# datastryio/weaviate

Measured on AMD Instinct MI355X. Metric: batched 10-NN QPS at recall@10≥0.95, 1M×128-d L2, on 1/2/4/8 MI355X, higher is better.
Workload: dtype f32 (f16 MFMA keys certified by an error bound, f32 reference-order re-rank)

## Files before the change

weaviate_amd/csrc/wv_api.hip:

```cpp
#include <hip/hip_runtime.h>
#include <hipcub/hipcub.hpp>

#include <algorithm>
#include <array>
#include <atomic>
#include <chrono>
#include <cmath>
#include <cstdio>
#include <cstdlib>
#include <condition_variable>
#include <cstring>
#include <mutex>
#include <string>
#include <vector>

#include "../../include/wvgpu.h"
#include "wv_device.h"

#include "wv_params.h"

extern "C" {
hipError_t wv_launch_bf_mfma(const wv::BfParams* p, hipStream_t s);
hipError_t wv_launch_bf_finalize(const wv::BfFinParams* p, hipStream_t s);
hipError_t wv_launch_bf_finalize_wide(const wv::BfFinParams* p, hipStream_t s);
// ... 567 lines not shown
        excl = ix->cexcl.as<uint64_t>();
        allow = nullptr;
    }
    if (ix->metric == WV_L2_SQUARED)
        HIP_TRY(wv_launch_h16_xns(xnorm, ntl * tile_rows, ix->h16_sx, ix->qscale.as<float>(), ix->xns.as<float>(), s));
    wv::H16Params hp{};
    hp.X = ximg;
    hp.rowidx = wd ? rowidx : nullptr;
    hp.Q = ix->qimg16.p;
    hp.xns = ix->xns.as<float>();
    hp.excl = excl;
    hp.allow = allow;
    hp.qscale = ix->qscale.as<float>();
    hp.sx = ix->h16_sx;
    hp.N = N;
    hp.nq = nq;
    hp.metric = ix->metric;
    hp.n_qblocks = nqb;
    hp.wide_rows = 128;
    hp.clean_tiles = wd ? 0 : rowidx ? N / wv::H_BN : allow ? 0 : std::min<uint64_t>(ix->clean_words, N / wv::H_BN);
    hp.locality = 1;
    wv::BfFinParams fp{};
    fp.X = ix->vecs.as<float>();
    fp.Q = d_q;
    fp.qnorm = ix->q_nrm2.as<float>();
    fp.xnorm_max = ix->maxnorm_host;
    fp.nq = nq;
    fp.D = ix->dim;
    fp.ldx = ix->ldx;
    fp.ldq = ix->dpad;
    fp.metric = ix->metric;
    fp.k = k;
    fp.id_base = ix->cfg.id_base;
    fp.out_ids = d_out_ids;
    fp.out_d = d_out_d;
    fp.out_n = d_out_n;
    fp.fail = ix->fail.as<int32_t>();
    fp.fail_thr = ix->fail_thr.as<float>();
    fp.bq = bq;
    fp.prod = prod;
    fp.kp = kp;
    fp.h16 = 1;
    hp.ns = ns;
    fp.qscale = ix->qscale.as<float>();
    fp.sx = ix->h16_sx;
    fp.ex_max = ix->h16_ex;
    fp.qres = ix->qres.as<float>();
    const bool wide = k > wv::FIN_KF;
    auto target = [&](uint64_t tiles) {
        uint64_t t = (uint64_t)ix->n_cus * wg_per_cu;
        if (wide) t = std::max<uint64_t>(t, (uint64_t)nqb * std::min<uint64_t>(tiles, (uint64_t)k + 2));
        return (int)std::min<uint64_t>(t, 1u << 30);
    };
    int sample = wv::H_SAMPLE;
    if (const char* e = std::getenv("WV_H16_SAMPLE")) sample = std::max(1, std::atoi(e));
    const bool seed = !wd && ntl >= 64 * (uint64_t)sample && !std::getenv("WV_H16_NO_SEED");
    const uint64_t nts = seed ? (ntl + sample - 1) / sample : 0;
    wv::BfSchedule ss{};
    if (seed) ss = wv::bf_schedule(nq, nts * wv::H_BN, target(nts), bq, wv::H_BN);
    const bool seed_lists = seed && !wide && !n_dev && k <= 64 &&
                            (uint64_t)ss.n_slots * wv::H_PROD * wv::BF_KP <= 256 && std::getenv("WV_H16_SEED_LISTS");
    const uint64_t ntl_main = seed_lists ? ntl - nts : ntl;
    wv::BfSchedule sch{};
    if (n_dev) {
        if (!wd || wide) return fail(WV_ESTATE, "run_h16: device-counted rows need the wide-D pass");
        const int S = std::max(1, target(ntl) / nqb);
        sch.bq = bq;
        sch.ntiles = (uint64_t)S;
        sch.units_per_block = 1;
        sch.n_blocks = nqb * S;
        sch.n_slots = S + 1;
    }
    if (wd && !wide && sch.n_blocks == 0) sch = wv::bf_schedule_aligned(nq, N, target(ntl), bq, tile_rows, false);
    if (sch.n_blocks == 0)
        sch = wv::bf_schedule(nq, seed_lists ? ntl_main * tile_rows : N, target(ntl_main), bq, tile_rows);
    if (wide && (uint64_t)sch.n_slots * prod * kp > (uint64_t)wv::FINW_NE)
        return fail(WV_ESTATE, "run_h16: too many lists for the wide finalize");
    const int out_slots = sch.n_slots + (seed_lists ? 1 : 0);
    HIP_TRY(ix->cand_d.ensure((size_t)nq * out_slots * prod * kp * 4));
    HIP_TRY(ix->cand_id.ensure((size_t)nq * out_slots * prod * kp * 4));
    auto seed_minima = [&](int stride) -> int {
        const uint64_t nt = (ntl + stride - 1) / stride;
        const wv::BfSchedule ms = wv::bf_schedule(nq, nt * wv::H_BN, target(nt), bq, wv::H_BN);
        HIP_TRY(ix->cand_d.ensure((size_t)nq * std::max(ms.n_slots * seed_prod, out_slots * prod * kp) * 4));
        hp.ntiles = ms.ntiles;
        hp.ntiles_real = ms.ntiles;
        hp.units_per_block = ms.units_per_block;
        hp.n_slots = ms.n_slots;
        hp.tile_stride = stride;
        hp.tile_base = 0;
        hp.tau = nullptr;
        hp.out_d = ix->cand_d.as<float>();
        hp.out_id = nullptr;
        HIP_TRY(wv_launch_bf_h16(&hp, ns, 1, s));
        wv::H16SeedParams sp{};
        sp.minima = ix->cand_d.as<float>();
        sp.n_slots = ms.n_slots;
        sp.ntiles = ms.ntiles;
        sp.units_per_block = ms.units_per_block;
        sp.nq = nq;
        sp.k = k;
        sp.metric = ix->metric;
        sp.D = ix->dim;
        sp.qscale = ix->qscale.as<float>();
        sp.sx = ix->h16_sx;
        sp.qnorm = ix->q_nrm2.as<float>();
        sp.xnorm_max = ix->maxnorm_host;
        sp.ex_max = ix->h16_ex;
        sp.qres = ix->qres.as<float>();
// ... 2 lines not shown
        sp.bq = bq;
        sp.prod = seed_prod;
        if (seed_lists) {
            HIP_TRY(wv_launch_h16_seed(&sp, s));
            HIP_TRY(ix->seed_d.ensure((size_t)nq * ss.n_slots * prod * kp * 4));
            HIP_TRY(ix->seed_id.ensure((size_t)nq * ss.n_slots * prod * kp * 4));
            hp.ntiles = ss.ntiles;
            hp.ntiles_real = ss.ntiles;
            hp.units_per_block = ss.units_per_block;
            hp.n_slots = ss.n_slots;
            hp.tile_stride = 1;
            hp.tile_base = ntl_main;
            hp.tau = ix->tau.as<float>();
            hp.out_d = ix->seed_d.as<float>();
            hp.out_id = ix->seed_id.as<uint32_t>();
            HIP_TRY(wv_launch_bf_h16(&hp, ns, 0, s));
            hp.tile_base = 0;
            hp.tau = nullptr;
            sp.minima = ix->seed_d.as<float>();
            sp.ids = ix->seed_id.as<uint32_t>();
            sp.n_slots = ss.n_slots;
            sp.ntiles = ss.ntiles;
            sp.units_per_block = ss.units_per_block;
            sp.prod = prod * kp;
            sp.out_d = ix->cand_d.as<float>();
            sp.out_id = ix->cand_id.as<uint32_t>();
            sp.out_slots = out_slots;
            sp.out_ntiles = sch.ntiles;
            sp.out_upb = sch.units_per_block;
        }
        HIP_TRY(wv_launch_h16_seed(&sp, s));
        return WV_OK;
    };
    if (seed) {
        TREC(6);
        int mult = 4;
        if (const char* e = std::getenv("WV_H16_LIST_MULT")) mult = std::max(1, std::atoi(e));
        if (int rc = seed_minima(seed_lists ? mult * sample : sample)) return rc;
        TREC(7);
    }
    hp.ntiles = sch.ntiles;
    hp.ntiles_real = ntl_main;
    hp.out_slots = seed_lists ? out_slots : 0;
    hp.units_per_block = sch.units_per_block;
    hp.n_slots = sch.n_slots;
    hp.n_dev = n_dev;
    hp.tile_stride = 1;
    hp.tau = nullptr;
    if (!seed) HIP_TRY(hipMemsetAsync(ix->gtau.p, 0xFF, (size_t)nq * 4, s));
    hp.gtau = ix->gtau.as<unsigned int>();
    hp.kth = k <= (wd ? 2 * kp : prod * kp) && !seed && !std::getenv("WV_H16_NO_RUNNING")
                 ? k
                 : 0;
    const char* xe = std::getenv("WV_H16_XSLOT");
    const bool xs_on = !xe || std::atoi(xe) != 0;
    if (xs_on && !wd && 2 * sch.n_slots <= 32 && k <= 2 * sch.n_slots) {
        const size_t gb = (size_t)nq * 2 * sch.n_slots * 4;
        HIP_TRY(ix->gslot.ensure(gb));
        HIP_TRY(hipMemsetAsync(ix->gslot.p, 0x7F, gb, s));
        hp.gslot = ix->gslot.as<float>();
        hp.xslot = 1;
        hp.kth = k;
    }
    if (hp.kth) {
        HIP_TRY(ix->marg.ensure((size_t)nq * 4));
        HIP_TRY(wv_launch_h16_margin(ix->metric, ix->dim, ix->q_nrm2.as<float>(), ix->qres.as<float>(),
                                     ix->maxnorm_host, ix->h16_ex, ix->h16_sx, ix->qscale.as<float>(), nq,
                                     ix->marg.as<float>(), s));
        hp.marg = ix->marg.as<float>();
    }
    hp.out_d = ix->cand_d.as<float>();
    hp.out_id = ix->cand_id.as<uint32_t>();
    const bool rotate = !wd && nqb >= 2 && sch.ntiles == ntl_main;
    if (rotate) hp.locality |= 2;
    if (int rc = block_order(ix, (uint64_t)nqb, sch, s, &hp.block_order, rotate)) return rc;
    TREC(0);
    HIP_TRY(wd ? wv_launch_bf_h16w(&hp, s) : wv_launch_bf_h16(&hp, ns, 0, s));
    TREC(1);
    if (rowidx && wide)
        HIP_TRY(wv_launch_remap_ids(ix->cand_id.as<uint32_t>(), nq, sch.n_slots, prod * kp, bq, sch.ntiles,
                                    sch.units_per_block, rowidx, N, n_dev, s));
    if (rowidx && !wide) {
        fp.rowidx = rowidx;
        fp.rowidx_n = N;
        fp.rowidx_ndev = n_dev;
    }
    fp.cand_d = ix->cand_d.as<float>();
    fp.cand_id = ix->cand_id.as<uint32_t>();
    fp.n_slots = out_slots;
    fp.extra_slot = seed_lists ? 1 : 0;
    fp.ntiles = sch.ntiles;
    fp.units_per_block = sch.units_per_block;
    HIP_TRY(wv_launch_h16_gtau(ix->gtau.as<unsigned int>(), nq, ix->h16_sx, ix->qscale.as<float>(), ix->tau.as<float>(),
                               s));
    fp.tau_in = ix->tau.as<float>();
    TREC(2);
    HIP_TRY(wide ? wv_launch_bf_finalize_wide(&fp, s) : wv_launch_bf_finalize(&fp, s));
    TREC(3);
    (void)fails;
    return WV_OK;
}

int queue_fbd(wv_index* ix, const float* d_q, int nq, int k, const uint64_t* d_allow, uint64_t allow_nbits,
              uint64_t allow_stride, uint64_t* d_out_ids, float* d_out_d, int32_t* d_out_n, hipStream_t s) {
    const uint64_t N = ix->n_rows;
    HIP_TRY(ix->fbd_list.ensure((size_t)nq * 4));
    HIP_TRY(ix->fbd_nf.ensure(16));
    HIP_TRY(ix->fbd_over.ensure((size_t)nq * 4));
    HIP_TRY(ix->fbd_cd.ensure((size_t)nq * wv::FB_CAP * 4));
// ... 2013 lines not shown
```

weaviate_amd/csrc/wv_h16.hip:

```cpp
#include "wv_device.h"
#include "wv_params.h"
#include "wv_topk.h"

#include <float.h>

#include "wv_h16_dev.h"

namespace wv {


constexpr bool min_steps_cover(int ns) {
    unsigned m = 0;
    for (int k = 0; k < ns; ++k) {
        if (k == 0) m |= 7u;
        else if (k <= 6) m |= 3u << (2 * k + 1);
        if (k == ns - 1)
            for (int r = ns <= 7 ? 2 * ns + 1 : 15; r < 16; ++r) m |= 1u << r;
    }
    return m == 0xFFFFu;
}

template <int NS, bool L2, bool SEED, bool XS = false>
__global__ __launch_bounds__(512, 1) void wv_bf_h16_kernel(H16Params p) {
    static_assert(min_steps_cover(NS), "the spread tile minima must cover all 16 keys of a half");
// ... 4 lines not shown
    using St = H16Stage<NS>;
    const int tid = threadIdx.x;
    const int lane = tid & 63;
    const int wave = __builtin_amdgcn_readfirstlane(tid >> 6);
    const int khalf = lane >> 5;
    const int l31 = lane & 31;
    const uint4* __restrict__ X = reinterpret_cast<const uint4*>(p.X);
    const uint4* __restrict__ Qg = reinterpret_cast<const uint4*>(p.Q);
    const bool has_allow = p.allow != nullptr;
    const float s = p.sx * p.qscale[0];
    int lb = (int)blockIdx.x;
    if ((p.locality & 1) && gridDim.x >= 8) {
        const int nwg = (int)gridDim.x, q8 = nwg / 8, r8 = nwg % 8, xcd = (int)blockIdx.x % 8;
        lb = (xcd < r8 ? xcd * (q8 + 1) : r8 * (q8 + 1) + (xcd - r8) * q8) + (int)blockIdx.x / 8;
    }
    if (p.block_order) lb = p.block_order[lb];
    const uint64_t u_first = (uint64_t)lb * p.units_per_block;
    uint64_t u_last = u_first + p.units_per_block;
    if (u_last > (uint64_t)p.n_qblocks * p.ntiles) u_last = (uint64_t)p.n_qblocks * p.ntiles;

    const uint32_t lds0 = lds_addr(lds);
#ifdef WV_H16_PRIO
    if (wave >= 4) __builtin_amdgcn_s_setprio(1);
#endif
    const int n_ops = (wave < St::IMG_U4 / 64 ? (St::IMG_U4 / 64 - 1 - wave) / WAVES + 1 : 0) +
                      ((wave == 0 && L2) ? 1 : 0);
    const uint32_t voff = (uint32_t)(wave * 1024 + lane * 16);

    constexpr int NIMG = St::IMG_U4 / 64 > WAVES ? 2 : 1;
    static_assert(St::IMG_U4 / 64 <= 2 * WAVES, "a wave moves at most two image KiB per tile");
    constexpr int OPT = NIMG + (L2 ? 1 : 0);
    const uint32_t ct_step = (uint32_t)p.tile_stride, ct_span = (uint32_t)(p.ntiles * (uint64_t)p.tile_stride);
    const uint32_t ct_end = (uint32_t)p.tile_base + ct_span;
    const uint32_t dst_first = lds0 + (uint32_t)(wave * 1024), dst_end = dst_first + (uint32_t)(NSTG * TPS * St::U4 * 16);
    uint32_t f_ct = 0, f_dst = dst_first;
    int f_left = 0;
    int f_now = 0;
    auto fill_op = [&](int i) {
        if (i < NIMG) {
            if (wave + WAVES * i < St::IMG_U4 / 64)
                glds16s(uniform_ptr(X + (uint64_t)f_ct * St::IMG_U4), voff + (uint32_t)(i * WAVES * 1024),
                        f_dst + (uint32_t)(i * WAVES * 1024));
        } else if (wave == 0) {
            glds4s(uniform_ptr(p.xns + (uint64_t)f_ct * H_BN), (uint32_t)(lane * 4), f_dst + St::IMG_U4 * 16);
        }
        if (i == OPT - 1) {
            f_ct += ct_step;
            if (f_ct >= ct_end) f_ct -= ct_span;
            f_dst += (uint32_t)(St::U4 * 16);
            if (f_dst == dst_end) f_dst = dst_first;
            --f_now;
        }
    };
    constexpr int OPK = (OPT * TPS + 2 * NS - 1) / (2 * NS);
    static_assert(OPT * TPS <= 2 * NS * OPK, "a burst fits the two halves after its barrier");
    constexpr bool DMA_IN_E = OPT * TPS > NS * OPK;
    auto dma_steps = [&](int half) {
        return [&, half](int k) {
#pragma unroll
            for (int o = 0; o < OPK; ++o) {
                const int e = (half * NS + k) * OPK + o;
                if (e < OPT * TPS && f_now > 0) fill_op(e % OPT);
            }
        };
    };
    auto no_dma = [](int) {};

    uint64_t shift = 0;
    auto phys = [&](uint64_t t) {
        const uint64_t v = t + shift;
        return v >= p.ntiles ? v - p.ntiles : v;
    };
    auto next_slot = [](int sl) { return sl + 1 == NSTG * TPS ? 0 : sl + 1; };
    const uint32_t clean32 = (uint32_t)(p.clean_tiles < 0xFFFFFFFFull ? p.clean_tiles : 0xFFFFFFFFull);
    const uint32_t full32 = (uint32_t)(p.N / H_BN < 0xFFFFFFFFull ? p.N / H_BN : 0xFFFFFFFFull);

    for (uint64_t u = u_first; u < u_last;) {
        const int qb = (int)(u / p.ntiles);
        const uint64_t t_begin = u % p.ntiles;
        uint64_t t_end = t_begin + (u_last - u);
        if (t_end > p.ntiles) t_end = p.ntiles;
        u += t_end - t_begin;
        const int slot = lb - bf_first_block(qb, p.ntiles, p.units_per_block);
        shift = (p.locality & 2) ? (uint64_t)qb * p.ntiles % p.units_per_block % p.ntiles : 0;
        const int jq0 = qb * BQ + wave * 64 + l31;
        const int jq1 = jq0 + 32;
        const uint64_t t_stop = t_end < p.ntiles_real ? t_end : p.ntiles_real;
        const int ntile = t_stop > t_begin ? (int)(t_stop - t_begin) : 0;

        uint4 bq0[NS], bq1[NS];
        {
            const uint64_t g0 = (uint64_t)qb * (BQ / 32) + 2 * wave;
#pragma unroll
            for (int st = 0; st < NS; ++st) {
                bq0[st] = Qg[(g0 * NS + st) * 64 + lane];
                bq1[st] = Qg[((g0 + 1) * NS + st) * 64 + lane];
            }
        }
        float tau0 = FLT_MAX, tau1 = FLT_MAX;
        if (!SEED && p.gtau) {
            if (jq0 < p.nq) tau0 = fminf(FLT_MAX, h16_key_dec(p.gtau[jq0]));
            if (jq1 < p.nq) tau1 = fminf(FLT_MAX, h16_key_dec(p.gtau[jq1]));
        } else if (p.tau) {
            if (jq0 < p.nq) tau0 = fminf(FLT_MAX, p.tau[jq0] * s);
            if (jq1 < p.nq) tau1 = fminf(FLT_MAX, p.tau[jq1] * s);
        }
        if (jq0 >= p.nq) tau0 = -__builtin_inff();
        if (jq1 >= p.nq) tau1 = -__builtin_inff();
        float marg0 = 0.f, marg1 = 0.f;
        if (!SEED && p.kth) {
            if (jq0 < p.nq) marg0 = p.marg[jq0];
            if (jq1 < p.nq) marg1 = p.marg[jq1];
        }
#pragma unroll
        for (int st = 0; st < NS; ++st) asm volatile("" ::"v"(bq0[st].x), "v"(bq1[st].x));
        asm volatile("" ::"v"(tau0), "v"(tau1), "v"(marg0), "v"(marg1));
        float l0d[BF_KP], l1d[BF_KP];
        uint32_t l0i[BF_KP], l1i[BF_KP];
#pragma unroll
        for (int i = 0; i < BF_KP; ++i) {
            l0d[i] = FLT_MAX; l1d[i] = FLT_MAX;
            l0i[i] = WV_NIL; l1i[i] = WV_NIL;
        }
        const float INF = __builtin_inff();
        floatx16 acc00, acc01, acc10, acc11;
        floatx16 xcn;
        uint4 an0, an1;
        auto head = [&](const uint4* img, int rb) {
            if (L2) {
                const float* xn = reinterpret_cast<const float*>(img + St::IMG_U4) + 32 * rb;
#pragma unroll
                for (int g4 = 0; g4 < 4; ++g4) {
                    const float4 v = *reinterpret_cast<const float4*>(xn + 4 * khalf + 8 * g4);
                    xcn[4 * g4] = v.x; xcn[4 * g4 + 1] = v.y; xcn[4 * g4 + 2] = v.z; xcn[4 * g4 + 3] = v.w;
                }
            }
            an0 = img[(rb * NS) * 64 + lane];
            if (NS > 1) an1 = img[(rb * NS + 1) * 64 + lane];
        };
        auto mfma_half = [&](const uint4* img, int rb, floatx16& accA, floatx16& accB, auto&& between, auto&& dma,
                             const uint4* nimg, int nrb) {
            floatx16 xc;
            if (L2) xc = xcn;
            else {
#pragma unroll
                for (int r = 0; r < 16; ++r) xc[r] = 0.f;
            }
            uint4 a[3];
            a[0] = an0;
            a[1] = an1;
#pragma unroll
            for (int k = 0; k < NS; ++k) {
                __builtin_amdgcn_sched_barrier(0);
#ifdef WV_H16_ABLATE_NO_LDS
                if (k + 2 < NS) { a[(k + 2) % 3] = bq1[k + 2]; a[(k + 2) % 3].x ^= (uint32_t)rb; }
#else
                if (k + 2 < NS) a[(k + 2) % 3] = img[(rb * NS + k + 2) * 64 + lane];
#endif
                if (k == (NS >= 2 ? NS - 2 : 0)) head(nimg, nrb);
                const half8 ak = __builtin_bit_cast(half8, a[k % 3]);
                accA = __builtin_amdgcn_mfma_f32_32x32x16_f16(ak, __builtin_bit_cast(half8, bq0[k]), k == 0 ? xc : accA,
                                                              0, 0, 0);
                accB = __builtin_amdgcn_mfma_f32_32x32x16_f16(ak, __builtin_bit_cast(half8, bq1[k]), k == 0 ? xc : accB,
                                                              0, 0, 0);
#ifndef WV_H16_XC_INPLACE
                if (k == 0) asm volatile("" ::"v"(xc));
#endif
                dma(k);
                between(k);
// ... 5 lines not shown

                if (k == 0) { mA = fminf(fminf(A[0], A[1]), A[2]); mB = fminf(fminf(B[0], B[1]), B[2]); }
                else if (k == 1) { mA = fminf(fminf(mA, A[3]), A[4]); mB = fminf(fminf(mB, B[3]), B[4]); }
                else if (k == 2) { mA = fminf(fminf(mA, A[5]), A[6]); mB = fminf(fminf(mB, B[5]), B[6]); }
                else if (k == 3) { mA = fminf(fminf(mA, A[7]), A[8]); mB = fminf(fminf(mB, B[7]), B[8]); }
                else if (k == 4) { mA = fminf(fminf(mA, A[9]), A[10]); mB = fminf(fminf(mB, B[9]), B[10]); }
                else if (k == 5) { mA = fminf(fminf(mA, A[11]), A[12]); mB = fminf(fminf(mB, B[11]), B[12]); }
                else if (k == 6) { mA = fminf(fminf(mA, A[13]), A[14]); mB = fminf(fminf(mB, B[13]), B[14]); }
                if (k == NS - 1) {
#pragma unroll
                    for (int r = NS <= 7 ? 2 * NS + 1 : 15; r < 16; ++r) { mA = fminf(mA, A[r]); mB = fminf(mB, B[r]); }
                }
                asm volatile("" : "+v"(mA), "+v"(mB));
            };
        };
        auto tile_ok = [&](uint32_t ct, uint64_t& okw) -> bool {
            if (ct < clean32) {
                okw = ~0ull;
                return false;
            }
            okw = tile_okw32(p, ct, full32, has_allow);
            return okw != ~0ull;
        };
        auto lane_ok = [&](uint32_t okh, int jq) -> uint32_t { return (jq < p.nq ? okh : 0u) >> (4 * khalf); };
        auto mask_half = [&](floatx16& A, floatx16& B, uint32_t oa, uint32_t ob) {
            constexpr uint32_t LANE_ROWS = 0x0F0F0F0Fu;
            if (__all((oa & ob & LANE_ROWS) == LANE_ROWS)) return;
#pragma unroll
            for (int r = 0; r < 16; ++r) {
                const int bit = (r & 3) + 8 * (r >> 2);
                A[r] = (oa >> bit) & 1u ? A[r] : INF;
                B[r] = (ob >> bit) & 1u ? B[r] : INF;
            }
        };
        auto min16 = [&](const floatx16& A) {
#ifdef WV_H16_ABLATE_NO_MIN
            return A[0];
#endif
            float m0 = fminf(fminf(A[0], A[1]), A[2]), m1 = fminf(fminf(A[3], A[4]), A[5]);
            float m2 = fminf(fminf(A[6], A[7]), A[8]), m3 = fminf(fminf(A[9], A[10]), A[11]);
            m0 = fminf(fminf(m0, A[12]), A[13]);
            m1 = fminf(fminf(m1, A[14]), A[15]);
            return fminf(fminf(m0, m1), fminf(m2, m3));
        };

        uint64_t okw = 0;
        bool need_mask = false;
        float pt0 = 0.f, pt1 = 0.f;
        auto refresh_pt = [&] {
            pt0 = fminf(__shfl_xor(l0d[BF_KP - 1], 32, 64), tau0);
            pt1 = fminf(__shfl_xor(l1d[BF_KP - 1], 32, 64), tau1);
        };
        refresh_pt();
        const int ia = (p.kth + 1) >> 1, ib = p.kth >> 1;
        auto publish = [&] {
            int va = ia - 1, vb = ib - 1;
            asm volatile("" : "+v"(va), "+v"(vb));
            float a0 = -FLT_MAX, a1 = -FLT_MAX, b0 = -FLT_MAX, b1 = -FLT_MAX;
#pragma unroll
            for (int i = 0; i < BF_KP; ++i) {
                a0 = va == i ? l0d[i] : a0;
                a1 = va == i ? l1d[i] : a1;
                b0 = vb == i ? l0d[i] : b0;
                b1 = vb == i ? l1d[i] : b1;
            }
            b0 = __shfl_xor(b0, 32, 64);
            b1 = __shfl_xor(b1, 32, 64);
            const float k0 = fmaxf(a0, b0), k1 = fmaxf(a1, b1);
            if (khalf == 0) {
                const float u4 = 4.f * 5.9604645e-08f;
                if (jq0 < p.nq && k0 < FLT_MAX) {
                    const float t = k0 + marg0;
                    atomicMin(&p.gtau[jq0], h16_key_enc(t + u4 * (fabsf(k0) + marg0)));
                }
                if (jq1 < p.nq && k1 < FLT_MAX) {
                    const float t = k1 + marg1;
                    atomicMin(&p.gtau[jq1], h16_key_enc(t + u4 * (fabsf(k1) + marg1)));
                }
            }
            if (jq0 < p.nq) tau0 = fminf(tau0, h16_key_dec(__atomic_load_n(&p.gtau[jq0], __ATOMIC_RELAXED)));
            if (jq1 < p.nq) tau1 = fminf(tau1, h16_key_dec(__atomic_load_n(&p.gtau[jq1], __ATOMIC_RELAXED)));
            refresh_pt();
        };
        const bool running = !SEED && p.kth > 0 && p.gtau != nullptr && !p.xslot;
        const bool xs = XS && !SEED && p.kth > 0;
        auto xslot_step = [&](bool rd, bool wr) {
            const int nv = 2 * p.n_slots;
            if (rd) {
                const int jq = khalf ? jq1 : jq0;
                int nvv = jq < p.nq ? nv : 0;
                asm volatile("" : "+v"(nvv));
                const float* g = p.gslot + (size_t)jq * nv;
                float v[32];
#pragma unroll
                for (int i = 0; i < 32; ++i)
                    v[i] = i < nvv ? __hip_atomic_load(g + i, __ATOMIC_RELAXED, __HIP_MEMORY_SCOPE_AGENT) : FLT_MAX;
#pragma unroll
                for (int size = 2; size <= 32; size <<= 1)
#pragma unroll
                    for (int stride = size >> 1; stride > 0; stride >>= 1)
#pragma unroll
                        for (int i = 0; i < 32; ++i) {
                            const int j = i ^ stride;
                            if (j > i) {
                                const float a = v[i], b = v[j];
                                const bool up = (i & size) == 0;
                                v[i] = up ? fminf(a, b) : fmaxf(a, b);
                                v[j] = up ? fmaxf(a, b) : fminf(a, b);
                            }
                        }
                int ve = p.kth - 1;
                asm volatile("" : "+v"(ve));
                float kv = FLT_MAX;
#pragma unroll
                for (int i = 0; i < 32; ++i) kv = i == ve ? v[i] : kv;
                const float mg = khalf ? marg1 : marg0;
                const float u4 = 4.f * 5.9604645e-08f;
                float b = kv < 1e30f ? kv + mg + u4 * (fabsf(kv) + mg) : FLT_MAX;
                if (jq < p.nq && b < FLT_MAX) atomicMin(&p.gtau[jq], h16_key_enc(b));
                const float bo = __shfl_xor(b, 32, 64);
                tau0 = fminf(tau0, khalf ? bo : b);
                tau1 = fminf(tau1, khalf ? b : bo);
                refresh_pt();
            }
            if (wr) {
                const int s2 = 2 * slot + khalf;
                if (jq0 < p.nq && l0d[0] < FLT_MAX)
                    __hip_atomic_store(p.gslot + (size_t)jq0 * nv + s2, l0d[0], __ATOMIC_RELAXED, __HIP_MEMORY_SCOPE_AGENT);
                if (jq1 < p.nq && l1d[0] < FLT_MAX)
                    __hip_atomic_store(p.gslot + (size_t)jq1 * nv + s2, l1d[0], __ATOMIC_RELAXED, __HIP_MEMORY_SCOPE_AGENT);
            }
        };
        auto extract_half = [&](float m0, float m1, floatx16& A, floatx16& B, uint32_t rb) -> bool {
#ifdef WV_H16_ABLATE_NO_EXTRACT
            if (m0 == 1234.5f) l0d[0] = m1 + pt0 + pt1;
            return false;
#endif
#ifdef WV_H16_ABLATE_NO_EVENTS
            float nev = -INF;
            asm volatile("" : "+v"(nev));
            const bool x0 = m0 <= fminf(fminf(l0d[BF_KP - 1], pt0), nev), x1 = m1 <= fminf(fminf(l1d[BF_KP - 1], pt1), nev);
#else
            const bool x0 = m0 <= fminf(l0d[BF_KP - 1], pt0), x1 = m1 <= fminf(l1d[BF_KP - 1], pt1);
#endif
            const bool any = __any(x0 || x1);
            if (__builtin_expect(any, 0)) {
                WV_DBG_COUNT(3)
                if (__any(x0)) min_extract(m0, x0, A, pt0, l0d, l0i, rb);
                if (__any(x1)) min_extract(m1, x1, B, pt1, l1d, l1i, rb);
            }
            return any;
        };
        const int xs1 = ntile / 8, xs2 = ntile / 4, xs3 = ntile / 2, xs4 = (3 * ntile) / 4;
        const uint64_t p0 = phys(t_begin);
        uint32_t ct = (uint32_t)p.tile_base + (uint32_t)p0 * ct_step;
        f_ct = ct;
        f_dst = dst_first;
        f_now = ntile < 2 * TPS ? ntile : 2 * TPS;
        f_left = ntile - f_now;
        const int ops_in_flight = n_ops * (ntile <= TPS ? 0 : ntile < 2 * TPS ? ntile - TPS : TPS);
#pragma unroll
        for (int j = 0; j < 2 * TPS; ++j) {
            if (f_now > 0) {
#pragma unroll
                for (int i = 0; i < OPT; ++i) fill_op(i);
            }
        }
        vm_wait(ops_in_flight);
        block_barrier();
        if (ntile > 0) {
            head(lds, 0);
            mfma_half(lds, 0, acc00, acc01, [](int) {}, no_dma, lds, 1);
            need_mask = tile_ok(ct, okw);
        }
        int slot_t = 0;
        int tj = 0;
        int xs_next = XS && xs ? xs1 : -1;
        for (int t = 0; t < ntile; ++t) {
            const uint32_t rb0 = ct * (uint32_t)H_BN + 4 * khalf;
            ct += ct_step;
            if (ct >= ct_end) ct -= ct_span;
            WV_DBG_COUNT(0)
            const uint4* img = lds + slot_t * St::U4;
            slot_t = next_slot(slot_t);
            const bool more = t + 1 < ntile;
            if (tj == TPS - 1 && more) {
                vm_wait(0);
                block_barrier();
#ifndef WV_H16_ABLATE_NO_FILL
                f_now = f_left < TPS ? f_left : TPS;
                f_left -= f_now;
#endif
            }
            tj = tj == TPS - 1 ? 0 : tj + 1;
            const bool mask_t = need_mask;
            const uint4* nimg = more ? lds + slot_t * St::U4 : img;
            if (mask_t) mask_half(acc00, acc01, lane_ok((uint32_t)okw, jq0), lane_ok((uint32_t)okw, jq1));
            float m0, m1;
#ifdef WV_H16_ABLATE_NO_MIN
            m0 = acc00[0]; m1 = acc01[0];
            mfma_half(img, 1, acc10, acc11, [](int) {}, dma_steps(0), nimg, 0);
#else
#ifdef WV_H16_FILL_DUP
            if (f_now > 0) mfma_half(img, 1, acc10, acc11, min_steps(acc00, acc01, m0, m1), dma_steps(0), nimg, 0);
            else mfma_half(img, 1, acc10, acc11, min_steps(acc00, acc01, m0, m1), no_dma, nimg, 0);
#else
            mfma_half(img, 1, acc10, acc11, min_steps(acc00, acc01, m0, m1), dma_steps(0), nimg, 0);
#endif
#endif
            bool grew = false;
            if constexpr (SEED) {
                l0d[0] = fminf(l0d[0], m0);
                l1d[0] = fminf(l1d[0], m1);
            } else {
                grew = extract_half(m0, m1, acc00, acc01, rb0);
            }
            if (mask_t)
                mask_half(acc10, acc11, lane_ok((uint32_t)(okw >> 32), jq0), lane_ok((uint32_t)(okw >> 32), jq1));
            if (more) {
#ifdef WV_H16_ABLATE_NO_MIN
                m0 = acc10[0]; m1 = acc11[0];
                if constexpr (DMA_IN_E) mfma_half(nimg, 0, acc00, acc01, [](int) {}, dma_steps(1), nimg, 1);
                else mfma_half(nimg, 0, acc00, acc01, [](int) {}, no_dma, nimg, 1);
#else
                if constexpr (DMA_IN_E) mfma_half(nimg, 0, acc00, acc01, min_steps(acc10, acc11, m0, m1), dma_steps(1), nimg, 1);
                else mfma_half(nimg, 0, acc00, acc01, min_steps(acc10, acc11, m0, m1), no_dma, nimg, 1);
#endif
                need_mask = tile_ok(ct, okw);
            } else {
                m0 = min16(acc10);
                m1 = min16(acc11);
            }
            if constexpr (SEED) {
                l0d[0] = fminf(l0d[0], m0);
                l1d[0] = fminf(l1d[0], m1);
            } else {
                grew = extract_half(m0, m1, acc10, acc11, rb0 + 32) || grew;
                if (running && (t & 15) == 15) publish();
                else if (grew) refresh_pt();
                if constexpr (XS) {
                    if (t == xs_next) {
                        xslot_step(t != xs1, t != xs4);
                        xs_next = t < xs2 && xs2 > t ? xs2 : t < xs3 && xs3 > t ? xs3 : t < xs4 && xs4 > t ? xs4 : -1;
                    }
                }
            }
        }
        vm_wait(0);
        block_barrier();

        if constexpr (SEED) {
            if (jq0 < p.nq) p.out_d[((size_t)jq0 * p.n_slots + slot) * H_PROD + khalf] = l0d[0];
            if (jq1 < p.nq) p.out_d[((size_t)jq1 * p.n_slots + slot) * H_PROD + khalf] = l1d[0];
            continue;
        }
        const size_t per_q = (size_t)(p.out_slots ? p.out_slots : p.n_slots) * H_PROD * BF_KP;
        if (jq0 < p.nq) {
            const size_t base = (size_t)jq0 * per_q + ((size_t)slot * H_PROD + khalf) * BF_KP;
#pragma unroll
            for (int i = 0; i < BF_KP; ++i) { p.out_d[base + i] = l0d[i]; p.out_id[base + i] = l0i[i]; }
        }
        if (jq1 < p.nq) {
            const size_t base = (size_t)jq1 * per_q + ((size_t)slot * H_PROD + khalf) * BF_KP;
#pragma unroll
            for (int i = 0; i < BF_KP; ++i) { p.out_d[base + i] = l1d[i]; p.out_id[base + i] = l1i[i]; }
        }
    }
}

template <int WR>
struct HWStage {
    static constexpr int RG = WR / 32;
    static constexpr int BN = 2 * WR;
    static constexpr int KC = WR == 64 ? HW_KC : HW_KC / 2;
    static constexpr int A_U4 = 2 * RG * KC * 64;
    static constexpr int B_U4 = 8 * KC * 64;
    static constexpr int U4 = A_U4 + B_U4;
    static constexpr int WORDS = BN / 64;
    static constexpr int EX_U4 = BN / 4 + WORDS / 2 * 2;
    static constexpr int OPS = 2 + KC;
};
constexpr int HW_STAGES = 3;

template <bool L2, int WR>
__global__ __launch_bounds__(512, 1) void wv_bf_h16w_kernel(H16Params p) {
    extern __shared__ uint4 lds[];
    using St = HWStage<WR>;
    constexpr int RG = St::RG, KC = St::KC, BN = St::BN;
    const int tid = threadIdx.x;
    const int lane = tid & 63;
    const int wave = __builtin_amdgcn_readfirstlane(tid >> 6);
    const int khalf = lane >> 5;
    const int l31 = lane & 31;
    const int rh = wave & 1, qq = wave >> 1;
    const int ns = p.ns, nch = ns / KC;
    const uint4* __restrict__ Qg = reinterpret_cast<const uint4*>(p.Q);
// ... 585 lines not shown
    if (n_dev) n = *n_dev;
    const uint64_t lo = w * 64;
    excl[w] = lo >= n ? ~0ull : (n - lo >= 64 ? 0ull : ~0ull << (n - lo));
}

hipError_t wv_launch_h16_compact_aux(const float* xnorm, const uint32_t* rowidx, uint64_t n, const uint32_t* n_dev,
                                     float* cxnorm, uint64_t* excl, uint64_t excl_words, hipStream_t s) {
    if (n) hipLaunchKernelGGL(wv_gather_f32_kernel, dim3((unsigned)((n + 255) / 256)), dim3(256), 0, s, xnorm, rowidx, n,
                              n_dev, cxnorm);
    hipLaunchKernelGGL(wv_excl_tail_kernel, dim3((unsigned)((excl_words + 255) / 256)), dim3(256), 0, s, excl, n,
                       n_dev, excl_words);
    return hipGetLastError();
}

hipError_t wv_launch_remap_ids(uint32_t* ids, int nq, int n_slots, int per_slot, int bq, uint64_t ntiles,
                               uint64_t units_per_block, const uint32_t* rowidx, uint64_t n_rows, const uint32_t* n_dev,
                               hipStream_t s) {
    if (nq == 0) return hipSuccess;
    hipLaunchKernelGGL(wv_remap_ids_kernel, dim3((unsigned)nq), dim3(64), 0, s, ids, nq, n_slots, per_slot, bq, ntiles,
                       units_per_block, rowidx, n_rows, n_dev);
    return hipGetLastError();
}

hipError_t wv_launch_absmax(const float* in, int ld, uint64_t n, int D, unsigned int* max_bits, hipStream_t s) {
    if (n == 0) return hipSuccess;
    uint64_t blocks = (n * (uint64_t)D + 255) / 256;
    if (blocks > 1024) blocks = 1024;
    hipLaunchKernelGGL(wv::wv_absmax_kernel, dim3((unsigned)blocks), dim3(256), 0, s, in, ld, n, D, max_bits);
    return hipGetLastError();
}

hipError_t wv_launch_h16_qscale(const float* part, int nparts, unsigned int* max_bits, float bsign, float* qscale,
                                hipStream_t s) {
    hipLaunchKernelGGL(wv::wv_h16_qscale_kernel, dim3(1), dim3(256), 0, s, part, nparts, max_bits, bsign, qscale);
    return hipGetLastError();
}

hipError_t wv_launch_h16_xns(const float* xnorm, uint64_t n, float sx, const float* qscale, float* xns, hipStream_t s) {
    if (n == 0) return hipSuccess;
    hipLaunchKernelGGL(wv::wv_h16_xns_kernel, dim3((unsigned)((n + 255) / 256)), dim3(256), 0, s, xnorm, n, sx, qscale,
                       xns);
    return hipGetLastError();
}

hipError_t wv_launch_bf_h16(const wv::H16Params* p, int ns, int seed, hipStream_t s) {
    const uint64_t total = (uint64_t)p->n_qblocks * p->ntiles;
    const unsigned nb = (unsigned)((total + p->units_per_block - 1) / p->units_per_block);
    if (nb == 0) return hipSuccess;
    if (ns < 1 || ns > wv::H_NS_MAX || !p->X || !p->Q || !p->excl || !p->qscale || p->tile_stride < 1 ||
        (p->out_slots && p->out_slots < p->n_slots) || (seed && (p->out_slots || p->tile_base)))
        return hipErrorInvalidValue;
    const bool l2 = p->metric == WV_METRIC_L2;
    if (l2 && !p->xns) return hipErrorInvalidValue;
    const size_t lds = (size_t)wv::H_STAGES * wv::H_TPS8 * (2 * ns * 64 + 17) * 16;
#define WV_H16_GO(NS, L, S)                                                                                    \
    if (!S && p->xslot)                                                                                        \
        hipLaunchKernelGGL((wv::wv_bf_h16_kernel<NS, L, false, true>), dim3(nb), dim3(512), lds, s, *p);       \
    else hipLaunchKernelGGL((wv::wv_bf_h16_kernel<NS, L, S>), dim3(nb), dim3(512), lds, s, *p);
#define WV_H16_LAUNCH(NS)                     \
    if (seed) {                               \
        if (l2) { WV_H16_GO(NS, true, true) } \
        else { WV_H16_GO(NS, false, true) }   \
    } else {                                  \
        if (l2) { WV_H16_GO(NS, true, false) } \
        else { WV_H16_GO(NS, false, false) }  \
    }
    switch (ns) {
        case 1: WV_H16_LAUNCH(1) break;
        case 2: WV_H16_LAUNCH(2) break;
        case 3: WV_H16_LAUNCH(3) break;
        case 4: WV_H16_LAUNCH(4) break;
        case 5: WV_H16_LAUNCH(5) break;
        case 6: WV_H16_LAUNCH(6) break;
        case 7: WV_H16_LAUNCH(7) break;
        default: WV_H16_LAUNCH(8) break;
    }
#undef WV_H16_LAUNCH
#undef WV_H16_GO
    return hipGetLastError();
}

hipError_t wv_launch_h16_margin(int metric, int D, const float* qnorm, const float* qres, float xnorm_max,
                                float ex_max, float sx, const float* qscale, int nq, float* marg, hipStream_t s) {
    if (nq == 0) return hipSuccess;
    hipLaunchKernelGGL(wv::wv_h16_margin_kernel, dim3((nq + 255) / 256), dim3(256), 0, s, metric, D, qnorm, qres,
                       xnorm_max, ex_max, sx, qscale, nq, marg);
    return hipGetLastError();
}

hipError_t wv_launch_h16_gtau(const unsigned int* gtau, int nq, float sx, const float* qscale, float* tau,
                              hipStream_t s) {
    if (nq == 0) return hipSuccess;
    hipLaunchKernelGGL(wv::wv_h16_gtau_kernel, dim3((nq + 255) / 256), dim3(256), 0, s, gtau, nq, sx, qscale, tau);
    return hipGetLastError();
}

hipError_t wv_launch_bf_h16w(const wv::H16Params* p, hipStream_t s) {
    const uint64_t total = (uint64_t)p->n_qblocks * p->ntiles;
    const unsigned nb = (unsigned)((total + p->units_per_block - 1) / p->units_per_block);
    if (nb == 0) return hipSuccess;
    if (p->ns < 2 * wv::HW_KC || p->ns > wv::HW_NS_MAX || p->ns % wv::HW_KC || !p->X || !p->Q || !p->excl ||
        p->tile_stride != 1 || p->tile_base != 0 || p->out_slots != 0)
        return hipErrorInvalidValue;
    const bool l2 = p->metric == WV_METRIC_L2;
    if (l2 && !p->xns) return hipErrorInvalidValue;
    if (p->wide_rows != 128) return hipErrorInvalidValue;
    using St = wv::HWStage<128>;
// ... 18 lines not shown
```

weaviate_amd/csrc/wv_h16_dev.h:

```cpp
#pragma once
#include "wv_device.h"
#include "wv_params.h"
#include "wv_topk.h"

#include <float.h>

namespace wv {

typedef _Float16 half8 __attribute__((ext_vector_type(8)));
typedef float floatx4 __attribute__((ext_vector_type(4)));

__device__ __forceinline__ uint32_t lds_addr(const void* p) {
    return (uint32_t)(uintptr_t)(const __attribute__((address_space(3))) void*)p;
}
__device__ __forceinline__ void glds16(const void* src, uint32_t lds_wave_base) {
    uint32_t keep;
    asm volatile("s_mov_b32 %0, m0\n\ts_mov_b32 m0, %2\n\ts_nop 0\n\tglobal_load_lds_dwordx4 %1, off\n\ts_mov_b32 m0, %0"
                 : "=&s"(keep) : "v"(src), "s"(lds_wave_base) : "memory");
}
__device__ __forceinline__ void glds16s(const void* sbase, uint32_t voff, uint32_t lds_wave_base) {
    uint32_t keep;
    asm volatile("s_mov_b32 %0, m0\n\ts_mov_b32 m0, %3\n\ts_nop 0\n\tglobal_load_lds_dwordx4 %1, %2\n\ts_mov_b32 m0, %0"
                 : "=&s"(keep) : "v"(voff), "s"(sbase), "s"(lds_wave_base) : "memory");
}
// ... 27 lines not shown
__device__ __forceinline__ void vm_wait(int n) {
    switch (n) {
        case 0: asm volatile("s_waitcnt vmcnt(0)" ::: "memory"); break;
        case 1: asm volatile("s_waitcnt vmcnt(1)" ::: "memory"); break;
        case 2: asm volatile("s_waitcnt vmcnt(2)" ::: "memory"); break;
        case 3: asm volatile("s_waitcnt vmcnt(3)" ::: "memory"); break;
        case 4: asm volatile("s_waitcnt vmcnt(4)" ::: "memory"); break;
        case 5: asm volatile("s_waitcnt vmcnt(5)" ::: "memory"); break;
        case 6: asm volatile("s_waitcnt vmcnt(6)" ::: "memory"); break;
        case 7: asm volatile("s_waitcnt vmcnt(7)" ::: "memory"); break;
        default: asm volatile("s_waitcnt vmcnt(8)" ::: "memory"); break;
    }
}
__device__ __forceinline__ void block_barrier() {
#ifdef WV_H16_ABLATE_NO_BARRIER
    asm volatile("s_waitcnt lgkmcnt(0)" ::: "memory");
#else
    asm volatile("s_waitcnt lgkmcnt(0)\n\ts_barrier" ::: "memory");
#endif
}

__device__ __forceinline__ uint64_t tile_okw(const H16Params& p, uint64_t tile, bool has_allow) {
    typedef const __attribute__((address_space(4))) uint64_t cu64;
    const uint32_t tl = __builtin_amdgcn_readfirstlane((uint32_t)tile);
    uint64_t okw = ~((cu64*)p.excl)[tl];
    if (has_allow) okw &= ((cu64*)p.allow)[tl];
    const uint64_t row0 = (uint64_t)tl * H_BN;
    if (row0 + H_BN > p.N) okw &= p.N > row0 ? ((1ull << (p.N - row0)) - 1) : 0ull;
    return okw;
}

__device__ __forceinline__ uint64_t tile_okw32(const H16Params& p, uint32_t tile, uint32_t full_tiles, bool has_allow) {
    typedef const __attribute__((address_space(4))) uint64_t cu64;
    const uint32_t tl = __builtin_amdgcn_readfirstlane(tile);
    uint64_t okw = ~((cu64*)p.excl)[tl];
    if (has_allow) okw &= ((cu64*)p.allow)[tl];
    if (tl >= full_tiles) {
        const uint64_t row0 = (uint64_t)tl * H_BN;
        okw &= p.N > row0 ? ((1ull << (p.N - row0)) - 1) : 0ull;
    }
    return okw;
}

template <int NS>
struct H16Stage {
    static constexpr int IMG_U4 = 2 * NS * 64;
    static constexpr int U4 = IMG_U4 + 16 + 1;
};
#ifndef WV_H16_TPS
#define WV_H16_TPS 3
#endif
constexpr int H_TPS8 = WV_H16_TPS;
constexpr int H_STAGES = 3;

}
```

weaviate_amd/csrc/wv_params.h:

```cpp
#pragma once
#include <stdint.h>

namespace wv {

constexpr int BF_BQ = 128;
constexpr int BF_BN = 128;
constexpr int BF_BK = 32;
constexpr int BF_LDT = 36;
constexpr int BF_KP = 8;
constexpr int BF_PROD = 4;
constexpr int FIN_KF = 32;
constexpr int BF_FAST_KMAX = 32;
constexpr int BF_WIDE_KMAX = 256;
constexpr int FINW_NE = 8192;
constexpr int FINW_KF = 1024;
constexpr int HNSW_EF_MAX = 512;

struct BfParams {
    const float* X;
    const float* Q;
    const float* xnorm;
    const uint64_t* tomb;
    const uint64_t* allow;
    const uint32_t* rowidx;
// ... 20 lines not shown
}

struct BfSchedule {
    int n_blocks, n_slots, bq;
    uint64_t ntiles, units_per_block;
};
inline BfSchedule bf_schedule(int nq, uint64_t N, int target_blocks, int bq = BF_BQ, int tile_rows = BF_BN) {
    BfSchedule s{};
    s.bq = bq;
    const uint64_t nqb = (uint64_t)(nq + bq - 1) / bq;
    s.ntiles = (N + tile_rows - 1) / tile_rows;
    const uint64_t total = nqb * s.ntiles;
    uint64_t nb = target_blocks > 0 ? (uint64_t)target_blocks : 1;
    if (nb > total) nb = total;
    s.units_per_block = (total + nb - 1) / nb;
    s.n_blocks = (int)((total + s.units_per_block - 1) / s.units_per_block);
    s.n_slots = (int)((s.ntiles + s.units_per_block - 1) / s.units_per_block) + 1;
    return s;
}
inline BfSchedule bf_schedule_aligned(int nq, uint64_t N, int target_blocks, int bq, int tile_rows,
                                      bool any_cost = false) {
    BfSchedule s{};
    s.bq = bq;
    const uint64_t nqb = (uint64_t)(nq + bq - 1) / bq;
    const uint64_t nt = (N + tile_rows - 1) / tile_rows;
    const uint64_t S = nqb ? (uint64_t)(target_blocks > 0 ? target_blocks : 1) / nqb : 0;
    if (nqb < 2 || S < 1 || nt < S) return s;
    const uint64_t U = (nt + S - 1) / S;
    const uint64_t flat = (nqb * nt + (uint64_t)target_blocks - 1) / (uint64_t)target_blocks;
    if (U > flat + flat / 64 && !any_cost) return s;
    s.units_per_block = U;
    s.ntiles = S * U;
    s.n_blocks = (int)(nqb * S);
    s.n_slots = (int)S + 1;
    return s;
}
#if defined(__HIPCC__)
__host__ __device__
#endif
inline int bf_first_block(uint64_t qb, uint64_t ntiles, uint64_t upb) { return (int)(qb * ntiles / upb); }
#if defined(__HIPCC__)
__host__ __device__
#endif
inline int bf_slots_of(uint64_t qb, uint64_t ntiles, uint64_t upb) {
    return (int)(((qb + 1) * ntiles - 1) / upb) - bf_first_block(qb, ntiles, upb) + 1;
}

constexpr int H_BN = 64;
constexpr int H_WAVES = 8;
constexpr int H_BQ = 512;
constexpr int H_PROD = 2;
constexpr int H_NS_MAX = 8;
constexpr int H_SAMPLE = 16;

#if defined(__HIPCC__)
__host__ __device__
#endif
inline uint64_t h16_index(uint64_t row, int k, int ns) {
    const uint64_t block = (row >> 5) * (uint64_t)ns + (uint64_t)(k >> 4);
    const uint64_t lane = (uint64_t)(((k >> 3) & 1) * 32) + (row & 31);
    return (block * 64 + lane) * 8 + (uint64_t)(k & 7);
}

#if defined(__HIPCC__)
__host__ __device__
#endif
inline uint64_t h16w_index(uint64_t row, int k, int ns) {
    return (row >> 4) * (uint64_t)ns * 256 + (uint64_t)(k >> 5) * 512 + (row & 15) * 32 + (uint64_t)(k & 31);
}

struct H16Params {
    const void* X;
    const void* Q;
    const float* xns;
    const uint64_t* excl;
    const uint64_t* allow;
    const float* tau;
    const float* qscale;
    float sx;
    uint64_t N;
    int nq, metric;
    int n_qblocks, n_slots;
    uint64_t ntiles, units_per_block;
    uint64_t ntiles_real;
    int tile_stride;
    uint64_t tile_base;
    int out_slots;
    uint64_t clean_tiles;
    int locality;
    const int* block_order;
    float* out_d;
    uint32_t* out_id;
    unsigned int* gtau;
    int kth;
    const float* marg;
    float* gslot;
    int xslot;
    int ns;
    int wide_rows;
    const uint32_t* rowidx;
    const uint32_t* n_dev;
};

constexpr int HW_BN = 256;
constexpr int HW_BQ = 256;
constexpr int HW_KC = 4;
// ... 209 lines not shown
```

Baseline: 4.123 million.

## Stream global tau into LDS via DMA slot and densify cross-slot exchange

In the cross-slot (XS) h16 brute-force kernel, the global per-query threshold is now prefetched into a per-wave LDS buffer through the existing asynchronous DMA schedule and folded into the running pruning threshold each tile group, replacing the separate running-gtau path. Slot minima are published at every exchange point, which now happens at eight evenly spaced points instead of four, and reads are thinned by a configurable sort stride. On the host, the seed sampling is coarsened when the XS path applies and the seed minimum is changed to a fixed tile count. Together these aim to tighten pruning earlier at lower exchange cost, in exchange for extra LDS, more atomic stores, and a sparser seed.

```diff
diff --git a/weaviate_amd/csrc/wv_api.hip b/weaviate_amd/csrc/wv_api.hip
--- a/weaviate_amd/csrc/wv_api.hip
+++ b/weaviate_amd/csrc/wv_api.hip
@@ -643,9 +643,15 @@
         if (wide) t = std::max<uint64_t>(t, (uint64_t)nqb * std::min<uint64_t>(tiles, (uint64_t)k + 2));
         return (int)std::min<uint64_t>(t, 1u << 30);
     };
+    const char* xe = std::getenv("WV_H16_XSLOT");
+    const bool xs_on = !xe || std::atoi(xe) != 0;
+    auto xs_fits = [&](const wv::BfSchedule& sc) { return xs_on && !wd && 2 * sc.n_slots <= 32 && k <= 2 * sc.n_slots; };
     int sample = wv::H_SAMPLE;
+    if (!wd && !n_dev && !std::getenv("WV_H16_SEED_LISTS") &&
+        xs_fits(wv::bf_schedule(nq, N, target(ntl), bq, tile_rows)))
+        sample = wv::H_SAMPLE_XS;
     if (const char* e = std::getenv("WV_H16_SAMPLE")) sample = std::max(1, std::atoi(e));
-    const bool seed = !wd && ntl >= 64 * (uint64_t)sample && !std::getenv("WV_H16_NO_SEED");
+    const bool seed = !wd && ntl >= (uint64_t)wv::H_SEED_MIN_TILES && !std::getenv("WV_H16_NO_SEED");
     const uint64_t nts = seed ? (ntl + sample - 1) / sample : 0;
     wv::BfSchedule ss{};
     if (seed) ss = wv::bf_schedule(nq, nts * wv::H_BN, target(nts), bq, wv::H_BN);
@@ -754,9 +760,7 @@
     hp.kth = k <= (wd ? 2 * kp : prod * kp) && !seed && !std::getenv("WV_H16_NO_RUNNING")
                  ? k
                  : 0;
-    const char* xe = std::getenv("WV_H16_XSLOT");
-    const bool xs_on = !xe || std::atoi(xe) != 0;
-    if (xs_on && !wd && 2 * sch.n_slots <= 32 && k <= 2 * sch.n_slots) {
+    if (xs_fits(sch)) {
         const size_t gb = (size_t)nq * 2 * sch.n_slots * 4;
         HIP_TRY(ix->gslot.ensure(gb));
         HIP_TRY(hipMemsetAsync(ix->gslot.p, 0x7F, gb, s));
diff --git a/weaviate_amd/csrc/wv_h16.hip b/weaviate_amd/csrc/wv_h16.hip
--- a/weaviate_amd/csrc/wv_h16.hip
+++ b/weaviate_amd/csrc/wv_h16.hip
@@ -80,15 +80,25 @@
             --f_now;
         }
     };
-    constexpr int OPK = (OPT * TPS + 2 * NS - 1) / (2 * NS);
-    static_assert(OPT * TPS <= 2 * NS * OPK, "a burst fits the two halves after its barrier");
-    constexpr bool DMA_IN_E = OPT * TPS > NS * OPK;
+    constexpr int NENT = OPT * TPS + (XS ? 1 : 0);
+    constexpr int OPK = (NENT + 2 * NS - 1) / (2 * NS);
+    static_assert(NENT <= 2 * NS * OPK, "a burst fits the two halves after its barrier");
+    constexpr bool DMA_IN_E = NENT > NS * OPK;
+    const uint32_t tau_dst = lds0 + (uint32_t)(NSTG * TPS * St::U4 * 16 + 256 * wave);
+    typedef __attribute__((address_space(3))) unsigned int lds_u32;
+    lds_u32* tau_lds = (lds_u32*)(reinterpret_cast<unsigned int*>(lds + NSTG * TPS * St::U4) + 64 * wave);
+    uint32_t tau_voff = 0;
+    int tj_now = 0;
     auto dma_steps = [&](int half) {
         return [&, half](int k) {
 #pragma unroll
             for (int o = 0; o < OPK; ++o) {
                 const int e = (half * NS + k) * OPK + o;
-                if (e < OPT * TPS && f_now > 0) fill_op(e % OPT);
+                if (e < OPT * TPS) {
+                    if (f_now > 0) fill_op(e % OPT);
+                } else if (XS && e == OPT * TPS) {
+                    if (tj_now == 0) glds4s_dev<0>(p.gtau, tau_voff, tau_dst);
+                }
             }
         };
     };
@@ -143,6 +153,10 @@
 #pragma unroll
         for (int st = 0; st < NS; ++st) asm volatile("" ::"v"(bq0[st].x), "v"(bq1[st].x));
         asm volatile("" ::"v"(tau0), "v"(tau1), "v"(marg0), "v"(marg1));
+        if constexpr (XS) {
+            tau_lds[lane] = 0xFFFFFFFFu;
+            tau_voff = 4u * (uint32_t)min(jq0 - l31 + lane, p.nq - 1);
+        }
         float l0d[BF_KP], l1d[BF_KP];
         uint32_t l0i[BF_KP], l1i[BF_KP];
 #pragma unroll
@@ -254,6 +268,13 @@
             pt1 = fminf(__shfl_xor(l1d[BF_KP - 1], 32, 64), tau1);
         };
         refresh_pt();
+        auto tau_apply = [&] {
+            const unsigned int w0 = tau_lds[l31], w1 = tau_lds[32 + l31];
+            tau0 = fminf(tau0, h16_key_dec(w0));
+            tau1 = fminf(tau1, h16_key_dec(w1));
+            pt0 = fminf(pt0, tau0);
+            pt1 = fminf(pt1, tau1);
+        };
         const int ia = (p.kth + 1) >> 1, ib = p.kth >> 1;
         auto publish = [&] {
             int va = ia - 1, vb = ib - 1;
@@ -284,10 +305,17 @@
             if (jq1 < p.nq) tau1 = fminf(tau1, h16_key_dec(__atomic_load_n(&p.gtau[jq1], __ATOMIC_RELAXED)));
             refresh_pt();
         };
-        const bool running = !SEED && p.kth > 0 && p.gtau != nullptr && !p.xslot;
+        const bool running = !XS && !SEED && p.kth > 0 && p.gtau != nullptr && !p.xslot;
         const bool xs = XS && !SEED && p.kth > 0;
-        auto xslot_step = [&](bool rd, bool wr) {
+        auto xslot_step = [&](bool rd) {
             const int nv = 2 * p.n_slots;
+            {
+                const int s2 = 2 * slot + khalf;
+                if (jq0 < p.nq && l0d[0] < FLT_MAX)
+                    __hip_atomic_store(p.gslot + (size_t)jq0 * nv + s2, l0d[0], __ATOMIC_RELAXED, __HIP_MEMORY_SCOPE_AGENT);
+                if (jq1 < p.nq && l1d[0] < FLT_MAX)
+                    __hip_atomic_store(p.gslot + (size_t)jq1 * nv + s2, l1d[0], __ATOMIC_RELAXED, __HIP_MEMORY_SCOPE_AGENT);
+            }
             if (rd) {
                 const int jq = khalf ? jq1 : jq0;
                 int nvv = jq < p.nq ? nv : 0;
@@ -325,13 +353,6 @@
                 tau1 = fminf(tau1, khalf ? b : bo);
                 refresh_pt();
             }
-            if (wr) {
-                const int s2 = 2 * slot + khalf;
-                if (jq0 < p.nq && l0d[0] < FLT_MAX)
-                    __hip_atomic_store(p.gslot + (size_t)jq0 * nv + s2, l0d[0], __ATOMIC_RELAXED, __HIP_MEMORY_SCOPE_AGENT);
-                if (jq1 < p.nq && l1d[0] < FLT_MAX)
-                    __hip_atomic_store(p.gslot + (size_t)jq1 * nv + s2, l1d[0], __ATOMIC_RELAXED, __HIP_MEMORY_SCOPE_AGENT);
-            }
         };
         auto extract_half = [&](float m0, float m1, floatx16& A, floatx16& B, uint32_t rb) -> bool {
 #ifdef WV_H16_ABLATE_NO_EXTRACT
@@ -353,7 +374,8 @@
             }
             return any;
         };
-        const int xs1 = ntile / 8, xs2 = ntile / 4, xs3 = ntile / 2, xs4 = (3 * ntile) / 4;
+        int xs_i = 0;
+        int rd_in = XS_READ_EVERY;
         const uint64_t p0 = phys(t_begin);
         uint32_t ct = (uint32_t)p.tile_base + (uint32_t)p0 * ct_step;
         f_ct = ct;
@@ -377,7 +399,7 @@
         }
         int slot_t = 0;
         int tj = 0;
-        int xs_next = XS && xs ? xs1 : -1;
+        int xs_next = XS && xs ? ntile / 16 : -1;
         for (int t = 0; t < ntile; ++t) {
             const uint32_t rb0 = ct * (uint32_t)H_BN + 4 * khalf;
             ct += ct_step;
@@ -393,8 +415,15 @@
                 f_now = f_left < TPS ? f_left : TPS;
                 f_left -= f_now;
 #endif
+                if constexpr (XS) {
+                    if (XS_READ_EVERY == 1 || --rd_in == 0) {
+                        tau_apply();
+                        rd_in = XS_READ_EVERY;
+                    }
+                }
             }
             tj = tj == TPS - 1 ? 0 : tj + 1;
+            tj_now = tj;
             const bool mask_t = need_mask;
             const uint4* nimg = more ? lds + slot_t * St::U4 : img;
             if (mask_t) mask_half(acc00, acc01, lane_ok((uint32_t)okw, jq0), lane_ok((uint32_t)okw, jq1));
@@ -442,8 +471,11 @@
                 else if (grew) refresh_pt();
                 if constexpr (XS) {
                     if (t == xs_next) {
-                        xslot_step(t != xs1, t != xs4);
-                        xs_next = t < xs2 && xs2 > t ? xs2 : t < xs3 && xs3 > t ? xs3 : t < xs4 && xs4 > t ? xs4 : -1;
+                        xslot_step(XS_SORT <= 1 || p.n_slots < XS_SORT || ((slot + xs_i) & (XS_SORT - 1)) == 0);
+                        do {
+                            ++xs_i;
+                            xs_next = xs_i < 8 ? (xs_i * ntile) >> 3 : -1;
+                        } while (xs_i < 8 && xs_next <= t);
                     }
                 }
             }
@@ -1135,7 +1167,9 @@
         return hipErrorInvalidValue;
     const bool l2 = p->metric == WV_METRIC_L2;
     if (l2 && !p->xns) return hipErrorInvalidValue;
-    const size_t lds = (size_t)wv::H_STAGES * wv::H_TPS8 * (2 * ns * 64 + 17) * 16;
+    const size_t lds = (size_t)wv::H_STAGES * wv::H_TPS8 * (2 * ns * 64 + 17) * 16 +
+                       (!seed && p->xslot ? (size_t)wv::H_XS_LDS : 0);
+    if (!seed && p->xslot && (!p->gtau || !p->gslot || !p->marg || p->kth < 1)) return hipErrorInvalidValue;
 #define WV_H16_GO(NS, L, S)                                                                                    \
     if (!S && p->xslot)                                                                                        \
         hipLaunchKernelGGL((wv::wv_bf_h16_kernel<NS, L, false, true>), dim3(nb), dim3(512), lds, s, *p);       \
diff --git a/weaviate_amd/csrc/wv_h16_dev.h b/weaviate_amd/csrc/wv_h16_dev.h
--- a/weaviate_amd/csrc/wv_h16_dev.h
+++ b/weaviate_amd/csrc/wv_h16_dev.h
@@ -103,5 +103,15 @@
 #endif
 constexpr int H_TPS8 = WV_H16_TPS;
 constexpr int H_STAGES = 3;
+#ifndef WV_H16_XS_SORT
+#define WV_H16_XS_SORT 4
+#endif
+#ifndef WV_H16_XS_READ_EVERY
+#define WV_H16_XS_READ_EVERY 1
+#endif
+constexpr int XS_SORT = WV_H16_XS_SORT;
+constexpr int XS_READ_EVERY = WV_H16_XS_READ_EVERY;
+static_assert(XS_SORT >= 1 && (XS_SORT & (XS_SORT - 1)) == 0 && XS_READ_EVERY >= 1, "see above");
+constexpr int H_XS_LDS = 8 * 256;
 
 }
diff --git a/weaviate_amd/csrc/wv_params.h b/weaviate_amd/csrc/wv_params.h
--- a/weaviate_amd/csrc/wv_params.h
+++ b/weaviate_amd/csrc/wv_params.h
@@ -96,6 +96,8 @@
 constexpr int H_PROD = 2;
 constexpr int H_NS_MAX = 8;
 constexpr int H_SAMPLE = 16;
+constexpr int H_SAMPLE_XS = 32;
+constexpr int H_SEED_MIN_TILES = 1024;
 
 #if defined(__HIPCC__)
 __host__ __device__
```

After: 4.271 million, median of 6. +3.6%, better.
